# githomin/sketches-py

Hardware: AMD Instinct MI355X
Metric: values ingested/sec (node) @1M streams eps=0.01; % of HBM roofline (higher is better)
Workload: dtype f64; 1 GPU; cfg3: 1000000 streams x 1000 values per GPU, eps=0.01, pareto, ingest + quantiles(.5,.9,.99); split=weak, streams_per_gpu=1000000, parallelism=stream-sharded x1, weak: every rank its own batch (no collective)

## Files before the change

### sketches-py_amd/csrc/gk_kernels.hip

```cpp
#include <hip/hip_runtime.h>
#include <hip/hip_ext.h>
#include <stdint.h>
#include <math.h>

#include <algorithm>
#include <atomic>
#include <limits>
#include <type_traits>

#include "gk_dev.h"
#include "gk_launch.h"
#include "gk_query.h"
#include "gk_state.h"
#include "gk_xor.h"

#define GK_PROF_NSEC 12
#ifndef GK_PROF_FIRST
#define GK_PROF_FIRST 1
#endif
#ifdef GK_PROF
__device__ unsigned long long gk_prof_acc[GK_PROF_NSEC];
__device__ __forceinline__ uint32_t gk_cycles() { return (uint32_t)__builtin_amdgcn_s_memtime(); }
#define GK_MARK(L, sec)                                      \
  do {                                                       \
    if (threadIdx.x == 0) {                                  \
      const uint32_t t_ = gk_cycles();                       \
      (L).prof[sec] += (uint32_t)(t_ - (L).prof_t);         \
      (L).prof_t = t_;                                       \
    }                                                        \
  } while (0)
#else
#define GK_MARK(L, sec) do { } while (0)
#endif
#ifdef GK_PROF
struct GKBigProf {
  unsigned long long acc[GK_PROF_NSEC];
  uint32_t t;
};
__device__ __forceinline__ GKBigProf& gk_big_prof() {
  __shared__ GKBigProf p;
  return p;
}
#define GK_BMARK(sec)                                        \
  do {                                                       \
    if (threadIdx.x == 0) {                                  \
      GKBigProf& p_ = gk_big_prof();                         \
      const uint32_t t_ = gk_cycles();                       \
      p_.acc[sec] += (uint32_t)(t_ - p_.t);                  \
      p_.t = t_;                                             \
    }                                                        \
  } while (0)
#define GK_WP_N 16
#define GK_WP_W 8
__device__ unsigned long long gk_wprof_acc[GK_WP_W][GK_WP_N];
struct GKWaveProf {
  unsigned long long acc[GK_WP_W][GK_WP_N];
  uint32_t t[GK_WP_W];
};
__device__ __forceinline__ GKWaveProf& gk_wave_prof() {
  __shared__ GKWaveProf p;
  return p;
}
#define GK_WMARK(pt)                                                   \
  do {                                                                 \
    if ((threadIdx.x & 63) == 0 && (threadIdx.x >> 6) < GK_WP_W) {     \
      GKWaveProf& p_ = gk_wave_prof();                                 \
      const int w_ = threadIdx.x >> 6;                                 \
      const uint32_t t_ = gk_cycles();                                 \
      p_.acc[w_][pt] += (uint32_t)(t_ - p_.t[w_]);                     \
      p_.t[w_] = t_;                                                   \
    }                                                                  \
  } while (0)
#else
#define GK_BMARK(sec) do { } while (0)
#define GK_WMARK(pt) do { } while (0)
#endif

#define GK_KEEP_BIT 0x40000000

__device__ __forceinline__ int gk_threshold(const GKState& st, int64_t n) {
  double t = floor(st.two_eps * (double)(n - 1));
  if (t > (double)GK_T_CLAMP) t = (double)GK_T_CLAMP;
  if (t < -1.0) t = -1.0;
  return (int)t;
}

__device__ __forceinline__ int clampi(int x, int lo, int hi) { return x < lo ? lo : (x > hi ? hi : x); }

__device__ __forceinline__ int clamp0(int x, int m) {
  int r;
  asm("v_med3_i32 %0, %1, 0, %2" : "=v"(r) : "v"(x), "v"(m));
  return r;
}

#define DPP_WAVE_SHR1 0x138
#define DPP_WAVE_SHL1 0x130

__device__ __forceinline__ int32_t wave_incl_max_i32(int32_t v) {
  v = max(v, __builtin_amdgcn_update_dpp(INT_MIN, v, DPP_ROW_SHR(1), 0xf, 0xf, false));
  v = max(v, __builtin_amdgcn_update_dpp(INT_MIN, v, DPP_ROW_SHR(2), 0xf, 0xf, false));
  v = max(v, __builtin_amdgcn_update_dpp(INT_MIN, v, DPP_ROW_SHR(4), 0xf, 0xf, false));
  v = max(v, __builtin_amdgcn_update_dpp(INT_MIN, v, DPP_ROW_SHR(8), 0xf, 0xf, false));
  v = max(v, __builtin_amdgcn_update_dpp(INT_MIN, v, DPP_ROW_BCAST15, 0xa, 0xf, false));
  v = max(v, __builtin_amdgcn_update_dpp(INT_MIN, v, DPP_ROW_BCAST31, 0xc, 0xf, false));
  return v;
}

__device__ __forceinline__ int wave_shr1(int v, int fill) {
  return __builtin_amdgcn_update_dpp(fill, v, DPP_WAVE_SHR1, 0xf, 0xf, false);
}

__device__ __forceinline__ int64_t wave_shr1_i64(int64_t v, int64_t fill) { return dpp64<DPP_WAVE_SHR1, 0xf>(v, fill); }

template <bool GLOBAL>
__device__ __forceinline__ void wsync() {
  if constexpr (GLOBAL) {
    __syncthreads();
  } else {
    __builtin_amdgcn_fence(__ATOMIC_RELEASE, "wavefront");
    __builtin_amdgcn_wave_barrier();
    __builtin_amdgcn_fence(__ATOMIC_ACQUIRE, "wavefront");
  }
}


template <int VPL>
__device__ __forceinline__ void gk_load_flush_values(double (&xv)[VPL], const double* pb, int p,
                                                     const double* xs, int cnt, int lane) {
  if (cnt <= 0) {
#pragma unroll
    for (int r = 0; r < VPL; ++r) xv[r] = 0.0;
    return;
  }
#pragma unroll
  for (int r = 0; r < VPL; ++r) {
    const int ic = min(lane + 64 * r, cnt - 1);
    const double* a = (ic < p) ? pb + ic : xs + (ic - p);
    xv[r] = *a;
  }
#pragma unroll
  for (int r = 0; r < VPL; ++r) xv[r] = (lane + 64 * r < cnt) ? xv[r] : 0.0;
}

struct GKHdrV {
  int32_t cls, slot, pend, E;
  int64_t n, xo, xe;
  double mn, mx;
};

template <bool MINMAX = true>
__device__ __forceinline__ void gk_hdr_issue(GKHdrV& h, const GKState& st, const int64_t* offs, int64_t s) {
  h.cls = st.cls[s];
  h.slot = st.slot[s];
  h.pend = st.pend[s];
  h.E = st.E[s];
  h.n = st.n[s];
  h.xo = offs[s];
  h.xe = offs[s + 1];
  if constexpr (MINMAX) {
    h.mn = st.mn[s];
    h.mx = st.mx[s];
  } else {
    h.mn = h.mx = 0.0;
  }
}

template <bool MINMAX>
__device__ __forceinline__ uint32_t gk_hdr1_issue(const GKState& st, const int64_t* offs, int64_t s, int lane) {
  constexpr int NW = MINMAX ? 14 : 10;
  const uint32_t* p = (const uint32_t*)(st.cls + s);
  if (lane == 1) p = (const uint32_t*)(st.slot + s);
  if (lane == 2) p = (const uint32_t*)(st.pend + s);
  if (lane == 3) p = (const uint32_t*)(st.E + s);
  if (lane >= 4) p = (const uint32_t*)(st.n + s) + (lane - 4);
  if (lane >= 6) p = (const uint32_t*)(offs + s) + (lane - 6);
  if constexpr (MINMAX) {
    if (lane >= 10) p = (const uint32_t*)(st.mn + s) + (lane - 10);
    if (lane >= 12) p = (const uint32_t*)(st.mx + s) + (lane - 12);
  }
  uint32_t w = 0;
  if (lane < NW) w = *p;
  return w;
}
__device__ __forceinline__ int32_t gk_hdr1_word(uint32_t w, int k) { return __builtin_amdgcn_readlane((int)w, k); }
__device__ __forceinline__ int64_t gk_hdr1_dword(uint32_t w, int k) {
  return (int64_t)(((uint64_t)(uint32_t)__builtin_amdgcn_readlane((int)w, k + 1) << 32) |
                   (uint32_t)__builtin_amdgcn_readlane((int)w, k));
}

__device__ __forceinline__ int64_t rfl64(int64_t v) {
  const int lo = __builtin_amdgcn_readfirstlane((int)(uint32_t)(uint64_t)v);
  const int hi = __builtin_amdgcn_readfirstlane((int)(uint32_t)((uint64_t)v >> 32));
  return (int64_t)(((uint64_t)(uint32_t)hi << 32) | (uint32_t)lo);
}

__device__ __forceinline__ GKRec* gk_table_ptr_cs(const GKState& st, int64_t s, int32_t c, int32_t slot) {
  return c == 0 ? st.tab[0] + s * (int64_t)st.cap[0] : st.tab[c] + (int64_t)slot * st.cap[c];
}

#define GK_SORT_LONG_MAX 4096
#ifndef GK_WG_MAX
#define GK_WG_MAX 64
#endif
#ifndef GK_WG_MIN_FLUSHES
#define GK_WG_MIN_FLUSHES 256
#endif
#define GK_WG_CAP 2048
#define GK_WG_PMAX 1024
#ifndef GK_PRESORT_REL
#define GK_PRESORT_REL 3
#endif
#ifndef GK_PRESORT_REL_WG
#define GK_PRESORT_REL_WG 5
#endif

__global__ __launch_bounds__(1024) void k_long_prep(GKState st, const int64_t* __restrict__ offs,
                                                    int32_t* __restrict__ list, int64_t* __restrict__ list_n,
                                                    const int32_t* __restrict__ count,
                                                    int64_t* __restrict__ list_ws, int64_t* __restrict__ list_b0,
                                                    int64_t ws_cap, int64_t* __restrict__ ws_need,
                                                    int32_t* __restrict__ wg_count, int wg_presort,
                                                    int32_t* __restrict__ go) {
  __shared__ uint64_t key[GK_SORT_LONG_MAX];
  const int cnt = *count;
  const int t = threadIdx.x;
  if (cnt > 1 && cnt <= GK_SORT_LONG_MAX) {
    int N = 2;
    while (N < cnt) N <<= 1;
    constexpr uint64_t LMAX = (1ull << 33) - 1;
    for (int i = t; i < N; i += 1024) {
      uint64_t k = ~0ull;
      if (i < cnt) {
        const int64_t s = list[i];
        uint64_t L = (uint64_t)(offs[s + 1] - offs[s]);
        if (L > LMAX) L = LMAX;
        k = ((LMAX - L) << 31) | (uint64_t)s;
      }
      key[i] = k;
    }
    __syncthreads();
    for (int k = 2; k <= N; k <<= 1) {
      for (int j = k >> 1; j > 0; j >>= 1) {
        for (int pp = t; pp < N / 2; pp += 1024) {
          const int i = ((pp & ~(j - 1)) << 1) | (pp & (j - 1));
          const int l = i + j;
          const uint64_t a = key[i], b = key[l];
          if ((a > b) == ((i & k) == 0)) {
            key[i] = b;
            key[l] = a;
          }
        }
        __syncthreads();
      }
    }
    for (int i = t; i < cnt; i += 1024) list[i] = (int32_t)(key[i] & 0x7fffffffu);
    __syncthreads();
  }
  for (int i = t; i < cnt; i += 1024) list_n[i] = st.n0[list[i]];
  if (!list_ws) return;
  __syncthreads();
  __shared__ int64_t part[1024];
  __shared__ unsigned long long nbmax;
  if (t == 0) nbmax = 0;
  __syncthreads();
  const int per = (cnt + 1023) / 1024;
  const int i0 = t * per, i1 = min(i0 + per, cnt);
  for (int i = i0; i < i1; ++i) {
    const int64_t s = list[i];
    int64_t nb = 0;
    if (st.cls[s] == 0) {
      const int64_t L = offs[s + 1] - offs[s];
      const int64_t need = st.P - (list_n[i] % st.P);
      nb = L >= need ? 1 + (L - need) / st.P : 0;
    }
    list_b0[i] = nb;
    atomicMax(&nbmax, (unsigned long long)nb);
  }
  __syncthreads();
  __shared__ int wk;
  if (wg_count) {
    if (t == 0) {
      int k = 0;
      while (k < cnt && k < GK_WG_MAX && list_b0[k] >= GK_WG_MIN_FLUSHES) ++k;
      if (!(st.cap[0] == GK_WG_CAP && st.P <= GK_WG_PMAX)) k = 0;
      *wg_count = k;
      wk = wg_presort ? k : 0;
    }
    __syncthreads();
  }
  const int64_t nb_min = (int64_t)(nbmax / (wg_count ? GK_PRESORT_REL_WG : GK_PRESORT_REL));
  int64_t mine = 0;
  for (int i = i0; i < i1; ++i) {
    if (list_b0[i] < nb_min || (wg_count && i >= wk)) list_b0[i] = 0;
    mine += list_b0[i];
  }
  part[t] = mine;
  __syncthreads();
  if (t == 0) {
    int64_t acc = 0;
    for (int k = 0; k < 1024; ++k) {
      const int64_t v = part[k];
      part[k] = acc;
      acc += v;
    }
    *ws_need = acc * st.P;
    list_b0[cnt] = acc;
  }
  __syncthreads();
  int64_t b = part[t];
  for (int i = i0; i < i1; ++i) {
    const int64_t nb = list_b0[i];
    list_b0[i] = b;
    list_ws[i] = (nb > 0 && (b + nb) * st.P <= ws_cap) ? b * st.P : -1;
    b += nb;
  }
  if (go) {
    __syncthreads();
    if (t == 0) {
      __threadfence();
      __hip_atomic_store(go, 1, __ATOMIC_RELEASE, __HIP_MEMORY_SCOPE_AGENT);
    }
  }
}

#ifndef GK_SL_BCAST
#define GK_SL_BCAST 1024
#endif

#define SL_BCAST_DEPTH 4
#ifndef SL_DEPTH
#define SL_DEPTH 7
#endif
// ... 1863 lines not shown
                                                   unsigned long long* __restrict__ work, int32_t* __restrict__ ctr) {
  const int lane = threadIdx.x;
  const int P = st.P;
  const BigBuf B = big_buf(ws + (size_t)blockIdx.x * ws_bytes, cap, gk_big_np(P));
  if (count_ptr) count = *count_ptr;
  if ((int64_t)blockIdx.x >= count) return;
  for (;;) {
    unsigned long long wv = 0;
    if (lane == 0) wv = atomicAdd(work, 1ull);
    const int64_t w = rfl64((int64_t)wv);
    if (w >= count) break;
    const int64_t s = list ? (int64_t)list[w] : w;
    if (__builtin_amdgcn_readfirstlane(st.cls[s]) != lcls) continue;
    int p = __builtin_amdgcn_readfirstlane(st.pend[s]);
    int E = __builtin_amdgcn_readfirstlane(st.E[s]);
    int64_t n = rfl64(st.n[s]);
    const int64_t xo = rfl64(offs[s]) + ((lcls > 0 && x) ? n - rfl64(st.n0[s]) : 0);
    const int64_t Lx = rfl64(offs[s + 1]) - xo;
    if (Lx <= 0 && !((force == 1 && p > 0) || (force == 2 && n > 0)) && !qs) continue;
    const bool over = !gk_count_ok(st, n + (Lx > 0 ? Lx : 0));
    const double smn = st.mn[s], smx = st.mx[s];
    GKRec* __restrict__ tab = gk_table_ptr(st, s);
    double* __restrict__ pb = st.pbuf + s * (int64_t)st.pmax;
    bool ok = !over && E <= cap - 1;
    if (ok) {
      for (int j = lane; j < E; j += 64) {
        const GKRec rc = tab[j];
        B.tv[0][j] = rc.v;
        B.tg[0][j] = rc.g;
        B.td[0][j] = rc.d;
      }
    }
    wsync<true>();
    int cur = 0;
    int64_t used = 0;
    int64_t need = P - (n % P);
    while (ok && used + need <= Lx) {
      big_load(B, pb, p, x + xo + used, p + (int)need, lane);
      n += need;
      const int nE = big_flush(B, cap, cur, E, p + (int)need, gk_threshold(st, n), lane);
      if (nE < 0) {
        ok = false;
        break;
      }
      E = nE;
      cur ^= 1;
      used += need;
      p = 0;
      need = P;
    }
    if (ok) {
      const int64_t rem = Lx - used;
      if ((force == 1 && p + rem > 0) || force == 2) {
        big_load(B, pb, p, rem > 0 ? x + xo + used : pb, p + (int)rem, lane);
        n += rem;
        const int nE = big_flush(B, cap, cur, E, p + (int)rem, gk_threshold(st, n), lane);
        if (nE < 0) {
          ok = false;
        } else {
          E = nE;
          cur ^= 1;
          p = 0;
        }
      } else {
        for (int64_t i = lane; i < rem; i += 64) pb[p + i] = x[xo + used + i];
        p += (int)rem;
        n += rem;
      }
    }
    if (!ok) {
      if (lane == 0) {
        if (over) {
          atomicAdd(&ctr[GK_CTR_FATAL], 1);
          atomicMax(&ctr[GK_CTR_FATAL + 1], (int)s);
        } else {
          const int k = atomicAdd(ovf_count, 1);
          ovf_list[k] = (int32_t)s;
        }
      }
      wsync<true>();
      continue;
    }
    const double* fv = cur ? B.tv[1] : B.tv[0];
    const int32_t* fg = cur ? B.tg[1] : B.tg[0];
    const int32_t* fd = cur ? B.td[1] : B.td[0];
    if (qs) wave_quantiles<1, 1>(fv, fg, fd, E, n, smn, smx, st, qs, nq, qmode, qout + s * (int64_t)nq, lane);
    for (int j = lane; j < E; j += 64) {
      GKRec rc;
      rc.v = fv[j];
      rc.g = fg[j];
      rc.d = fd[j];
      tab[j] = rc;
    }
    if (lane == 0) {
      st.n[s] = n;
      st.E[s] = E;
      st.pend[s] = p;
    }
    wsync<true>();
  }
}

#define SMALL_CAP GK_SMALL_CAP
#define GK_SMALL_LX_MAX (((int64_t)1 << 31) - ((int64_t)1 << 15))
#ifndef GK_SMALL_WAVES
#define GK_SMALL_WAVES 7
#endif
#ifndef GK_SMALL_RANK_MAX
#define GK_SMALL_RANK_MAX 16
#endif
__device__ __forceinline__ void gk_lds_order() { __asm__ volatile("" ::: "memory"); }

#ifndef GK_DUP
#define GK_DUP 0
#endif
#define GK_DUPG(g) ((GK_DUP >> (g)) & 1)
template <typename T>
__device__ __forceinline__ void dup_ld(const T* p) {
  const uint32_t a = (uint32_t)(uintptr_t)p;
  if constexpr (sizeof(T) == 16) {
    __attribute__((ext_vector_type(4))) uint32_t w;
    __asm__ volatile("ds_read_b128 %0, %1\n\ts_waitcnt lgkmcnt(0)" : "=v"(w) : "v"(a) : "memory");
  } else if constexpr (sizeof(T) == 8) {
    __attribute__((ext_vector_type(2))) uint32_t w;
    __asm__ volatile("ds_read_b64 %0, %1\n\ts_waitcnt lgkmcnt(0)" : "=v"(w) : "v"(a) : "memory");
  } else {
    uint32_t w;
    __asm__ volatile("ds_read_b32 %0, %1\n\ts_waitcnt lgkmcnt(0)" : "=v"(w) : "v"(a) : "memory");
  }
}
template <typename T>
__device__ __forceinline__ void dup_st(T* p, T v) {
  static_assert(sizeof(T) == 8, "8-byte stores only");
  unsigned long long u;
  __builtin_memcpy(&u, &v, 8);
  *(volatile unsigned long long*)p = u;
}

__device__ __forceinline__ int pidx(int i) { return i + (i >> 5); }
#define SMALL_TVN (SMALL_CAP + (SMALL_CAP >> 5) + 4)


#define GK_SMALL_TRASH (SMALL_CAP + 1)
static_assert(SMALL_CAP == 128, "k_ingest_small is laid out for the 128-entry class (K = 2 entries per lane)");
template <int VPL>
struct SmallLDS {
  alignas(16) double mv[64 * VPL + 64 + 2];
  alignas(16) double tv[SMALL_TVN];
  alignas(16) int2 tgd[SMALL_CAP + 2];
  union {
    alignas(16) int2 gi[SMALL_TVN];
    int32_t mi[64 * VPL + 2];
  };
#ifdef GK_PROF
  unsigned long long prof[GK_PROF_NSEC];
  uint32_t prof_t;
#endif
};

static_assert(SMALL_CAP + (SMALL_CAP >> 5) + 4 == 136, "gi zeroing covers 136 records");
static_assert(sizeof(int32_t) * (64 * 2 + 2) <= sizeof(int2) * 136, "mi fits in the records");
__device__ __forceinline__ void small_zero_counts(int2* gi, int lane) {
  typedef uint32_t gk_v4u __attribute__((ext_vector_type(4)));
  gk_v4u z;
  __asm__ volatile("v_mov_b64 %0, 0" : "=v"(z.xy));
  __asm__ volatile("v_mov_b64 %0, 0" : "=v"(z.zw));
  int l7 = lane & 7;
  __asm__ volatile("" : "+v"(l7));
  ((gk_v4u*)gi)[lane] = z;
  ((uint2*)gi)[128 + l7] = make_uint2(z.x, z.y);
}

__device__ __forceinline__ void small_pad(double* tv, int E, int lane) {
  tv[pidx(min(E + lane, SMALL_CAP - 1))] = __longlong_as_double(0x7ff0000000000000LL);
}

struct CsDiv {
  int cs;
  uint32_t m;
  __device__ __forceinline__ int div(int a) const { return (int)(__umul24((uint32_t)a, m) >> 23); }
  __device__ __forceinline__ int rem(int a, int q) const { return a - (int)__umul24((uint32_t)q, (uint32_t)cs); }
};

struct CsMagicTable {
  uint32_t m[256];
  constexpr CsMagicTable() : m() {
    for (uint32_t c = 1; c < 256; ++c) m[c] = ((1u << 23) + c - 1u) / c;
  }
};
__constant__ CsMagicTable gk_cs_magic = CsMagicTable();

__device__ __forceinline__ CsDiv make_csdiv(int T) {
  CsDiv c;
  c.cs = T > 1 ? T : 1;
  c.m = c.cs < 256 ? gk_cs_magic.m[c.cs] : 1u;
  return c;
}

__device__ __forceinline__ uint32_t gd_pack(int g, int d) { return __builtin_amdgcn_perm((uint32_t)d, (uint32_t)g, 0x05040100u); }
__device__ __forceinline__ int gd_g(uint32_t w) { return (int)(w & 0xffffu); }
__device__ __forceinline__ int gd_d(uint32_t w) { return (int)(w >> 16); }

template <int VPL, int DUPG = -1>
__device__ __forceinline__ void small_put(SmallLDS<VPL>& L, int pos, double v, int g, int d) {
  L.tv[pidx(pos)] = v;
  L.tgd[pos] = make_int2(g, d);
  if constexpr (DUPG >= 0 && GK_DUPG(DUPG)) {
    dup_st(&L.tv[pidx(pos)], v);
    dup_st(&L.tgd[pos], make_int2(g, d));
  }
}

__device__ __forceinline__ int gi_ob(int x) { return x & 0xff; }
__device__ __forceinline__ int gi_mb(int x) { return (x >> 8) & 0xff; }
__device__ __forceinline__ int gi_k(int x) { return (x >> 16) & 0xff; }
__device__ __forceinline__ int gi_m(int x) { return (int)((uint32_t)x >> 24); }

template <int VPL, bool NOTAIL = false>
__device__ __forceinline__ void small_emit(SmallLDS<VPL>& L, bool in_gap, const CsDiv& cd, double x, int2 gi,
                                           int rk, bool valid) {
  const int k = gi_k(gi.x);
  if constexpr (NOTAIL) {
    small_put<VPL, 8>(L, (valid && rk >= k) ? gi_ob(gi.x) + rk - k : GK_SMALL_TRASH, x, 1, gi.y);
    return;
  }
  const int q = cd.div(rk);
  const int rr = cd.rem(rk, q);
  const int pos = gi_ob(gi.x) + (in_gap ? rk - k : q);
  const bool keep = valid && (in_gap ? rk >= k : (rr == cd.cs - 1 || rk == gi_m(gi.x) - 1));
  small_put<VPL, 8>(L, keep ? pos : GK_SMALL_TRASH, x, in_gap ? 1 : rr + 1, in_gap ? gi.y : 0);
}

template <int J>
__device__ __forceinline__ int lane_xor_i32(int v, int lane) {
  return lane_xor_dpp<J>(v, lane);
}

template <int J>
__device__ __forceinline__ double lane_xor_f64(double v, int lane) {
  typedef int gk_v2i __attribute__((ext_vector_type(2)));
  const gk_v2i a = __builtin_bit_cast(gk_v2i, v);
  gk_v2i r;
  r.x = lane_xor_i32<J>(a.x, lane);
  r.y = lane_xor_i32<J>(a.y, lane);
  return __builtin_bit_cast(double, r);
}

template <int X, int LB>
__device__ __forceinline__ void cx_stage2(double (&a)[2], int lane) {
  const bool lower = (lane & LB) == 0;
  if constexpr (X == LB && (X == 16 || X == 32)) {
    typedef int gk_v2i __attribute__((ext_vector_type(2)));
#pragma unroll
    for (int r = 0; r < 2; ++r) {
      const gk_v2i v = __builtin_bit_cast(gk_v2i, a[r]);
      gk_v2i A, B;
      if constexpr (X == 16) {
        const auto lo = __builtin_amdgcn_permlane16_swap(v.x, v.x, false, false);
        const auto hi = __builtin_amdgcn_permlane16_swap(v.y, v.y, false, false);
        A.x = (int)lo[0]; B.x = (int)lo[1]; A.y = (int)hi[0]; B.y = (int)hi[1];
      } else {
        const auto lo = __builtin_amdgcn_permlane32_swap(v.x, v.x, false, false);
        const auto hi = __builtin_amdgcn_permlane32_swap(v.y, v.y, false, false);
        A.x = (int)lo[0]; B.x = (int)lo[1]; A.y = (int)hi[0]; B.y = (int)hi[1];
      }
      const double da = __builtin_bit_cast(double, A), db = __builtin_bit_cast(double, B);
      a[r] = ((db < da) == lower) ? db : da;
    }
    return;
  }
#pragma unroll
  for (int r = 0; r < 2; ++r) {
    const double p = lane_xor_f64<X>(a[r], lane);
    const bool take = (p < a[r]) == lower;
    a[r] = take ? p : a[r];
  }
}

template <int J>
__device__ __forceinline__ void half_cleaners2(double (&a)[2], int lane) {
  cx_stage2<J, J>(a, lane);
  if constexpr (J > 1) half_cleaners2<J / 2>(a, lane);
}

template <int KB>
__device__ __forceinline__ void sort_runs2(double (&a)[2], int lane) {
  if constexpr (KB > 2) sort_runs2<KB / 2>(a, lane);
  cx_stage2<KB - 1, KB / 2>(a, lane);
  if constexpr (KB >= 4) half_cleaners2<KB / 4>(a, lane);
}

__device__ __forceinline__ void sort128_2(double (&a)[2], int lane) {
  sort_runs2<64>(a, lane);
  {
    const double p0 = lane_xor_f64<63>(a[1], lane);
    const double p1 = lane_xor_f64<63>(a[0], lane);
    const bool t0 = p0 < a[0];
    const bool t1 = a[1] < p1;
    a[0] = t0 ? p0 : a[0];
    a[1] = t1 ? p1 : a[1];
  }
  half_cleaners2<32>(a, lane);
}

#define GK_PS_R 16

// ... 586 lines not shown
template <int VPL>
__device__ __attribute__((noinline)) double small_quantiles(SmallLDS<VPL>& L, int E, int64_t n, double mn, double mx,
                                                            double inv_eps, double eps, double qv, int qe, int qmode,
                                                            int lane) {
  const bool valid = (qv >= 0.0 && qv <= 1.0);
  if (n == 0 || E == 0) return gk_nan();
  if ((double)n < inv_eps)
    return valid ? percentile_linear_at(E, qv, [&](int i) { return L.tv[pidx(i)]; }) : gk_nan();
  const double spread_d = floor(eps * (double)(n - 1));
  const int myi = n < ((int64_t)1 << 30) ? small_rank_count<int32_t>(L, E, n, spread_d, qv, qe, lane)
                                         : small_rank_count<int64_t>(L, E, n, spread_d, qv, qe, lane);
  if (!valid) return gk_nan();
  if (myi == 0) return mn;
  if (myi < E) return L.tv[pidx(myi - 1)];
  return (qmode == 0) ? mx : L.tv[pidx(E - 1)];
}

#ifndef GK_FS_DEPTH
#define GK_FS_DEPTH 2
#endif
#define GK_SWORK_IDX 128
#ifndef GK_FS_LAG_DEFAULT
#define GK_FS_LAG_DEFAULT 256
#endif
#ifndef GK_FS_DRAIN
#define GK_FS_DRAIN 1
#endif
#ifndef GK_FS_SPIN_MAX
#define GK_FS_SPIN_MAX (1 << 16)
#endif

template <int DEPTH = GK_FS_DEPTH>
__device__ __forceinline__ void fused_stats_role(const GKState& st, const double* __restrict__ x,
                                                 const int64_t* __restrict__ offs,
                                                 unsigned long long* __restrict__ work, int part, int lgp,
                                                 int64_t count, int pace, int lag, int lane) {
  const int64_t pbeg = (count * part) >> lgp, pend = (count * (part + 1)) >> lgp;
  const int64_t nb = (pend - pbeg + 63) / 64;
  unsigned long long* __restrict__ swork = work + GK_SWORK_IDX + 16 * part;
  unsigned long long* __restrict__ iwork = work + 16 * part;
  const double2* __restrict__ dummy = (const double2*)st.rtab;
  for (;;) {
    unsigned long long v = 0;
    if (lane == 0) v = atomicAdd(swork, 1ull);
    const int64_t b = rfl64((int64_t)v);
    if (b >= nb) break;
    if (pace) {
      const int64_t want = min((b + 1) * 64 + (int64_t)lag, pend - pbeg);
      for (int spin = 0; spin < GK_FS_SPIN_MAX; ++spin) {
        unsigned long long got = 0;
        if (lane == 0) got = __hip_atomic_load(iwork, __ATOMIC_RELAXED, __HIP_MEMORY_SCOPE_AGENT);
        if (rfl64((int64_t)got) >= want) break;
        __builtin_amdgcn_s_sleep(8);
      }
    }
    const int64_t s = (int64_t)((int)(pbeg + b * 64) + lane);
    const bool live = s < pend;
    const int64_t xo = live ? offs[s] : 0;
    int64_t rem = live ? offs[s + 1] - xo : 0;
    if (rem > GK_STATS_LONG) rem = 0;
    const bool act = rem > 0;
    int64_t n = 0;
    double mn = 0, mx = 0, sm = 0, av = 0;
    if (act) {
      n = st.n0[s];
      mn = st.mn[s];
      mx = st.mx[s];
      sm = st.sum[s];
      av = st.avg[s];
    }
    const int64_t peel = (act && (((uintptr_t)(x + xo)) & 8)) ? 1 : 0;
    if (peel) {
      gk_stat_step(x[xo], n, sm, av, mn, mx);
      --rem;
    }
    const double* p = x + xo + peel;
    const int64_t nch = rem / 8;
    int64_t maxch = nch;
#pragma unroll
    for (int o = 32; o > 0; o >>= 1) maxch = max(maxch, (int64_t)__shfl_xor(maxch, o, 64));
    const double2* __restrict__ p2 = (const double2*)p;
    int64_t nlo = act ? n : INT64_MAX, nhi = act ? n : INT64_MIN;
#pragma unroll
    for (int o = 32; o > 0; o >>= 1) {
      nlo = min(nlo, (int64_t)__shfl_xor(nlo, o, 64));
      nhi = max(nhi, (int64_t)__shfl_xor(nhi, o, 64));
    }
    const int64_t nu = rfl64(nlo);
    const bool uni = nu == rfl64(nhi) && nu >= 0 && nu + 8 * maxch + 8 < st.rtab_n;
    double2 ring[DEPTH][4];
#pragma unroll
    for (int d = 0; d < DEPTH; ++d) {
      const double2* src = (d < nch) ? p2 + d * 4 : dummy;
#pragma unroll
      for (int j = 0; j < 4; ++j) ring[d][j] = src[j];
    }
    auto walk = [&](auto tab) {
      constexpr bool TAB = decltype(tab)::value;
      for (int64_t c0 = 0; c0 < maxch; c0 += DEPTH) {
#pragma unroll
        for (int d = 0; d < DEPTH; ++d) {
          const int64_t c = c0 + d;
          if (c < nch) {
            const double* __restrict__ rt = st.rtab + (nu + 8 * c + 1);
#pragma unroll
            for (int k = 0; k < 8; ++k) {
              const double v = (k & 1) ? ring[d][k >> 1].y : ring[d][k >> 1].x;
              const double rc = TAB ? rt[k] : 1.0 / (double)(n + 1 + k);
              sm = sm + v;
              av = av + (v - av) * rc;
              if (v < mn) mn = v;
              if (v > mx) mx = v;
            }
            n += 8;
          }
          const int64_t nx = c + DEPTH;
          const double2* src = (nx < nch) ? p2 + nx * 4 : dummy;
#pragma unroll
          for (int j = 0; j < 4; ++j) ring[d][j] = src[j];
        }
      }
    };
    if (uni) walk(std::true_type{});
    else walk(std::false_type{});
    const int tail = (int)(rem - nch * 8);
    for (int k = 0; k < tail; ++k) gk_stat_step(p[nch * 8 + k], n, sm, av, mn, mx);
    if (act) {
      st.mn[s] = mn;
      st.mx[s] = mx;
      st.sum[s] = sm;
      st.avg[s] = av;
    }
  }
}

#ifdef GK_TIMELINE
#define GK_TL_MAXS (1 << 20)
#define GK_TL_MAXW 16384
__device__ unsigned long long gk_tl_wave[5 * GK_TL_MAXW];
__device__ unsigned long long gk_tl_sbeg[GK_TL_MAXS];
__device__ unsigned long long gk_tl_send[GK_TL_MAXS];
#endif
template <int VPL, bool FS, int W = GK_SMALL_WAVES>
__global__ __launch_bounds__(64, W) void k_ingest_small(GKState st, const double* __restrict__ x,
                                                     const int64_t* __restrict__ offs, int64_t count, int force,
                                                     int32_t* __restrict__ ovf_count, int32_t* __restrict__ ovf_list,
                                                     const double* __restrict__ qs, int nq,
                                                     double* __restrict__ qout, int qmode,
                                                     unsigned long long* __restrict__ work, int nstat,
                                                     int fs_pace, int fs_lag) {
  __shared__ __attribute__((aligned(16))) SmallLDS<VPL> L;
  const int lane = threadIdx.x;
  const int P = st.P;
#ifdef GK_PROF
  if (lane == 0) {
    for (int i = 0; i < GK_PROF_NSEC; ++i) L.prof[i] = 0;
    L.prof_t = gk_cycles();
  }
#endif
  uint32_t hv = 0;
#ifndef GK_WORK_PARTS
#define GK_WORK_PARTS 8
#endif
#ifndef GK_WORK_CHUNK
#define GK_WORK_CHUNK 2
#endif
  static_assert((GK_WORK_PARTS & (GK_WORK_PARTS - 1)) == 0, "a power of two");
  int lgp = 0;
  while ((2 << lgp) <= GK_WORK_PARTS && (2u << lgp) <= gridDim.x) ++lgp;
  const int part = (int)(blockIdx.x & ((1u << lgp) - 1u));
#ifdef GK_TIMELINE
  if (lane == 0 && blockIdx.x < GK_TL_MAXW) {
    gk_tl_wave[5 * blockIdx.x] = __builtin_amdgcn_s_memrealtime();
    gk_tl_wave[5 * blockIdx.x + 3] = __builtin_amdgcn_s_memtime();
  }
#endif
  if (FS && (int)blockIdx.x < nstat) fused_stats_role(st, x, offs, work, part, lgp, count, fs_pace, fs_lag, lane);
#ifdef GK_TIMELINE
  if (lane == 0 && blockIdx.x < GK_TL_MAXW) gk_tl_wave[5 * blockIdx.x + 1] = __builtin_amdgcn_s_memrealtime();
#endif
  const int64_t pbeg = (count * part) >> lgp, pend = (count * (part + 1)) >> lgp;
  const double qpre = (qs && lane < nq) ? qs[lane] : 0.0;
  int64_t cur = 0, cend = 0;
  auto grab = [&]() -> int64_t {
    if (cur >= cend) {
      unsigned long long v = 0;
      if (lane == 0) v = atomicAdd(work + 16 * part, (unsigned long long)GK_WORK_CHUNK);
      cur = pbeg + rfl64((int64_t)v);
      cend = min(cur + GK_WORK_CHUNK, pend);
      if (cur >= pend) return count;
    }
    return cur++;
  };
  int64_t w = grab();
  if (w < count) hv = gk_hdr1_issue<!FS>(st, offs, w, lane);
#ifdef GK_PROF
  bool prof_done_any = false;
#endif
  for (; w < count;) {
    const int64_t s = w;
    const int64_t wn = grab();
    const int32_t scls = gk_hdr1_word(hv, 0);
    const int32_t sslot = gk_hdr1_word(hv, 1);
    int p = gk_hdr1_word(hv, 2);
    int E = gk_hdr1_word(hv, 3);
    int64_t n = gk_hdr1_dword(hv, 4);
    const int64_t xo = gk_hdr1_dword(hv, 6);
    const int64_t xe = gk_hdr1_dword(hv, 8);
    const double smn = __longlong_as_double(FS ? GK_QMARK_MIN : gk_hdr1_dword(hv, 10));
    const double smx = __longlong_as_double(FS ? GK_QMARK_MAX : gk_hdr1_dword(hv, 12));
    if (wn < count) hv = gk_hdr1_issue<!FS>(st, offs, wn, lane);
    w = wn;
    if (scls != 0) continue;
#ifdef GK_TIMELINE
    if (lane == 0 && s < GK_TL_MAXS) gk_tl_sbeg[s] = __builtin_amdgcn_s_memrealtime();
#endif
    const int64_t Lx = xe - xo;
    if (Lx <= 0 && !((force == 1 && p > 0) || (force == 2 && n > 0)) && !qs) continue;
    GKRec* __restrict__ tab = gk_table_ptr_cs(st, s, scls, sslot);
    double* __restrict__ pb = st.pbuf + s * (int64_t)st.pmax;
    bool ok = E <= SMALL_CAP - 1 && gk_count_ok(st, n + (Lx > 0 ? Lx : 0)) && Lx < GK_SMALL_LX_MAX;
    if (ok) {
      const int4* __restrict__ t4 = (const int4*)tab;
      int4 rc[SMALL_CAP / 64];
#pragma unroll
      for (int r = 0; r < SMALL_CAP / 64; ++r)
        rc[r] = (lane + 64 * r < E) ? t4[lane + 64 * r] : make_int4(0, 0, 0, 0);
#pragma unroll
      for (int r = 0; r < SMALL_CAP / 64; ++r) {
        const int j = lane + 64 * r;
        if (j < E) {
          L.tv[pidx(j)] = __hiloint2double(rc[r].y, rc[r].x);
          L.tgd[j] = make_int2(rc[r].z, rc[r].w);
        }
      }
      small_pad(L.tv, E, lane);
      small_zero_counts(L.gi, lane);
    }
    wsync<false>();
    GK_MARK(L, 0);

    bool flushed = false;
    bool final_done = false;
    const int L32 = (int)Lx;
    int used = 0;
    const int need0 = P - (int)(n % P);
    int need = need0;
    const double nm1c = (double)(n - 1);
    int fl = 0;
    int tT = 0;
    uint32_t tM = 0;
    auto plan_t = [&]() {
      const int k = min(need0 + (fl + lane) * P, L32);
      tT = (int)(st.two_eps * (nm1c + (double)k));
      const uint32_t cs = (uint32_t)max(tT, 1);
      tM = cs < 256u ? ((1u << 23) + cs - 1u) / cs : 1u;
    };
    const double* const xs = x ? x + xo : pb;
    double xv[VPL];
#pragma unroll
    for (int r = 0; r < VPL; ++r) xv[r] = 0.0;
    while (ok) {
      const bool autof = need <= L32 - used;
      int nadd;
      if (autof) {
        nadd = need;
      } else {
        nadd = L32 - used;
        if (!((force == 1 && p + nadd > 0) || force == 2)) break;
      }
      const int cnt = p + nadd;
      if (!flushed) gk_load_flush_values<VPL>(xv, pb, p, xs, cnt, lane);
      const int nused = used + nadd;
      const int navail = autof ? min(P, L32 - nused) : 0;
      double xn[VPL];
      auto prefetch = [&]() {
        const __amdgpu_buffer_rsrc_t rs =
            __builtin_amdgcn_make_buffer_rsrc((void*)(xs + nused), 0, navail * (int)sizeof(double), 0x00020000);
#pragma unroll
        for (int r = 0; r < VPL; ++r)
          xn[r] = __builtin_bit_cast(double, __builtin_amdgcn_raw_buffer_load_b64(rs, (lane + 64 * r) * 8, 0, 0));
      };
      if ((fl & 63) == 0) plan_t();
      n += nadd;
      const int T = __builtin_amdgcn_readlane(tT, fl & 63);
      CsDiv cd;
      cd.cs = max(T, 1);
      cd.m = (uint32_t)__builtin_amdgcn_readlane((int)tM, fl & 63);
      ++fl;
      GK_MARK(L, (GK_PROF_FIRST == 2 ? !flushed : (GK_PROF_FIRST && !prof_done_any)) ? 11 : 8);
      int nE;
      if constexpr (SMALL_CAP > 128)
        nE = E <= 127 ? flush_small<VPL, 2>(L, E, xv, cnt, T, cd, lane, prefetch)
                      : flush_small<VPL, 4>(L, E, xv, cnt, T, cd, lane, prefetch);
      else
        nE = flush_small<VPL, 2>(L, E, xv, cnt, T, cd, lane, prefetch);
      if (nE < 0) {
        n -= nadd;
        ok = false;
        break;
      }
      E = nE;
      used = nused;
      p = 0;
      need = P;
      flushed = true;
#pragma unroll
      for (int r = 0; r < VPL; ++r) xv[r] = xn[r];
      GK_MARK(L, 10);
      if (!autof) {
        final_done = true;
        break;
      }
    }
    if (ok && !final_done) {
      const int rem = L32 - used;
      if (flushed) {
#pragma unroll
        for (int r = 0; r < VPL; ++r)
          if (lane + 64 * r < rem) pb[lane + 64 * r] = xv[r];
      } else {
        for (int i = lane; i < rem; i += 64) pb[p + i] = xs[used + i];
      }
      p += rem;
      n += rem;
    }
    auto write_back = [&]() {
      double v[2];
      int2 gd[2];
#pragma unroll
      for (int r = 0; r < 2; ++r) {
        v[r] = L.tv[pidx(lane + 64 * r)];
        gd[r] = L.tgd[lane + 64 * r];
      }
#pragma unroll
      for (int r = 0; r < 2; ++r)
        if (lane + 64 * r < E) ((int4*)tab)[lane + 64 * r] = make_int4(__double2loint(v[r]), __double2hiint(v[r]), gd[r].x, gd[r].y);
      if (lane == 0) {
        st.n[s] = n;
        st.E[s] = E;
        st.pend[s] = p;
      }
    };
    if (!ok) {
      if (flushed) write_back();
      if (lane == 0) {
        const int k = atomicAdd(ovf_count, 1);
        ovf_list[k] = (int32_t)s;
      }
      wsync<false>();
      continue;
    }
    if (qs) {
      for (int q0 = 0; q0 < nq; q0 += 64) {
        int ql = lane;
        __asm__ volatile("" : "+v"(ql));
        const double qv = nq <= 64 ? qpre : ((q0 + ql < nq) ? qs[q0 + ql] : 0.0);
        const double r = small_quantiles<VPL>(L, E, n, smn, smx, st.inv_eps, st.eps, qv, min(nq - q0, 64), qmode, lane);
        if (q0 + ql < nq) qout[s * (int64_t)nq + q0 + ql] = r;
      }
    }
    write_back();
    wsync<false>();
    GK_MARK(L, 9);
#ifdef GK_TIMELINE
    if (lane == 0 && s < GK_TL_MAXS) gk_tl_send[s] = __builtin_amdgcn_s_memrealtime();
#endif
#ifdef GK_PROF
    prof_done_any = true;
#endif
  }
  if (FS && GK_FS_DRAIN) fused_stats_role(st, x, offs, work, part, lgp, count, fs_pace, fs_lag, lane);
#ifdef GK_PROF
  if (lane == 0)
    for (int i = 0; i < GK_PROF_NSEC; ++i) atomicAdd(&gk_prof_acc[i], L.prof[i]);
#endif
#ifdef GK_TIMELINE
  if (lane == 0 && blockIdx.x < GK_TL_MAXW) {
    gk_tl_wave[5 * blockIdx.x + 2] = __builtin_amdgcn_s_memrealtime();
    gk_tl_wave[5 * blockIdx.x + 4] = __builtin_amdgcn_s_memtime();
  }
#endif
}

#define GK_MAX_DEV 64
template <typename Q>
static int per_device(std::atomic<int> (&cache)[GK_MAX_DEV], Q query) {
  int dev = 0;
  (void)hipGetDevice(&dev);
  std::atomic<int>& c = cache[(unsigned)dev % GK_MAX_DEV];
  int v = c.load(std::memory_order_relaxed);
  if (v <= 0) {
    v = query(dev);
    if (v <= 0) v = 1;
    c.store(v, std::memory_order_relaxed);
  }
  return v;
}

static int num_cu() {
  static std::atomic<int> cache[GK_MAX_DEV];
  return per_device(cache, [](int dev) {
    hipDeviceProp_t prop;
    return hipGetDeviceProperties(&prop, dev) == hipSuccess && prop.multiProcessorCount > 0 ? prop.multiProcessorCount
                                                                                           : 256;
  });
}

int gk_num_cu() { return num_cu(); }

int gk_wg_early_ok() { return num_cu() >= 2 * GK_WG_MAX; }

template <int CAP, int VPL>
static hipError_t launch_ingest_t(const GKState& st, const double* x, const int64_t* offs,
                                  const int32_t* list, int64_t count, const int32_t* count_ptr, int lcls,
                                  int force, int cap,
                                  unsigned char* ws, size_t ws_bytes, int64_t ws_blocks,
                                  int32_t* ovf_count, int32_t* ovf_list, const GKQuery& q,
                                  unsigned long long* work, const int32_t* prio, const int32_t* prio_count,
                                  const double* psort, const int64_t* prio_ws, const int32_t* prio_skip, hipStream_t stream,
                                  const GKPoolDev& pool, int pmode) {
  if (count <= 0 && !count_ptr) return hipSuccess;
  if (!work) return hipErrorInvalidValue;
  int64_t grid;
  if (CAP > 0) {
    static std::atomic<int> occ_cache[GK_MAX_DEV];
    const int occ = per_device(occ_cache, [](int) {
      int o = 0;
      (void)hipOccupancyMaxActiveBlocksPerMultiprocessor(&o, k_ingest<CAP, VPL>, 64, 0);
      return o;
    });
    grid = (int64_t)num_cu() * occ;
  } else {
    grid = ws_blocks;
  }
  if (!prio && !count_ptr && grid > count) grid = count;
  if (grid < 1) grid = 1;
  hipLaunchKernelGGL((k_ingest<CAP, VPL>), dim3((unsigned)grid), dim3(64), 0, stream, st, x, offs, list,
                     count, count_ptr, lcls, force, cap, ws, ws_bytes, ovf_count, ovf_list, q.qs, q.nq, q.out,
                     q.mode, work, prio, prio_count, psort, prio_ws, prio_skip, pool, pmode);
  return hipGetLastError();
}

template <int CAP>
static hipError_t launch_ingest_vpl(int vpl, const GKState& st, const double* x, const int64_t* offs,
                                    const int32_t* list, int64_t count, const int32_t* count_ptr, int lcls,
                                    int force, int cap, unsigned char* ws,
                                    size_t ws_bytes, int64_t ws_blocks, int32_t* ovf_count, int32_t* ovf_list,
                                    const GKQuery& q, unsigned long long* work, const int32_t* prio,
                                    const int32_t* prio_count, const double* psort, const int64_t* prio_ws, const int32_t* prio_skip,
                                    hipStream_t stream, const GKPoolDev& pool, int pmode) {
#define GK_L(V) launch_ingest_t<CAP, V>(st, x, offs, list, count, count_ptr, lcls, force, cap, ws, ws_bytes, ws_blocks, \
                                        ovf_count, ovf_list, q, work, prio, prio_count, psort, prio_ws, prio_skip, stream, \
                                        pool, pmode)
  switch (vpl) {
    case 1: return GK_L(1);
    case 2: return GK_L(2);
    case 4: return GK_L(4);
    case 8: return GK_L(8);
    case 16: return GK_L(16);
    default: return hipErrorInvalidValue;
  }
#undef GK_L
}

template <int VPL>
static hipError_t launch_ingest_small(const GKState& st, const double* x, const int64_t* offs, const int32_t* list,
                                      int64_t count, int force, int32_t* ovf_count, int32_t* ovf_list,
                                      const GKQuery& q, unsigned long long* work, int fused_stats,
                                      hipStream_t stream, hipEvent_t ev0, hipEvent_t ev1) {
  if (count <= 0) return hipSuccess;
  if (!work) return hipErrorInvalidValue;
  const bool fs_launch = fused_stats > 0 && x && !list;
  static std::atomic<int> occ_cache[2][2][GK_MAX_DEV];
  auto occ_of = [&](bool fs, bool w6) -> int {
    return per_device(occ_cache[fs][w6], [fs, w6](int) {
      int o = 0;
      if (fs) {
        if (w6) (void)hipOccupancyMaxActiveBlocksPerMultiprocessor(&o, k_ingest_small<VPL, true, 6>, 64, 0);
        else (void)hipOccupancyMaxActiveBlocksPerMultiprocessor(&o, k_ingest_small<VPL, true>, 64, 0);
      } else {
        if (w6) (void)hipOccupancyMaxActiveBlocksPerMultiprocessor(&o, k_ingest_small<VPL, false, 6>, 64, 0);
        else (void)hipOccupancyMaxActiveBlocksPerMultiprocessor(&o, k_ingest_small<VPL, false>, 64, 0);
      }
      return o;
    });
  };
  auto full_grid = [&](bool w6) -> int64_t {
    int64_t g = (int64_t)num_cu() * occ_of(fs_launch, w6);
    return std::max<int64_t>(1, std::min<int64_t>(g, count));
  };
  static const int w_env = getenv("GK_SMALL_W") ? atoi(getenv("GK_SMALL_W")) : 0;
  static const int few_rounds = getenv("GK_FEW_ROUNDS") ? atoi(getenv("GK_FEW_ROUNDS")) : 4;
  int64_t grid = full_grid(false);
  const int64_t rounds7 = (count + grid - 1) / grid;
  const bool w6 = w_env ? w_env == 6 : (GK_SMALL_WAVES != 6 && rounds7 <= few_rounds);
  if (w6) grid = full_grid(true);
  int nstat = 0;
  if (fs_launch) {
    const int64_t want = std::max<int64_t>(1, (int64_t)num_cu() * fused_stats / 8);
    nstat = (int)(grid < want ? grid : want);
  }
  const int pace = nstat > 0 && grid >= 4 * (int64_t)nstat && grid >= 8 * GK_WORK_PARTS ? 1 : 0;
  static const int lag = getenv("GK_FS_LAG") ? atoi(getenv("GK_FS_LAG")) : GK_FS_LAG_DEFAULT;
  if (list) return hipErrorInvalidValue;
#define GK_SMALL_LAUNCH(FS_, W_)                                                                              \
  hipExtLaunchKernelGGL((k_ingest_small<VPL, FS_, W_>), dim3((unsigned)grid), dim3(64), 0, stream, ev0, ev1, 0, st, x, \
                        offs, count, force, ovf_count, ovf_list, q.qs, q.nq, q.out, q.mode, work, nstat, pace, lag)
  if (nstat > 0) {
    if (w6) GK_SMALL_LAUNCH(true, 6);
    else GK_SMALL_LAUNCH(true, GK_SMALL_WAVES);
  } else {
    if (w6) GK_SMALL_LAUNCH(false, 6);
    else GK_SMALL_LAUNCH(false, GK_SMALL_WAVES);
// ... 135 lines not shown
```

Before: 181.9 billion values/s.

## Software-pipeline stream headers, work grabs and first value chunk across iterations

Restructures the small-ingest loop so the next stream's work-counter atomic, header load and first block of input values are issued while the current stream is still being processed, hiding their latency. Header base pointers and quantile probes are staged in LDS, and work indices are narrowed to 32-bit atomics. Skipped streams no longer `continue` early, so the control flow changes. This adds register pressure and more complex state that could cost occupancy, and the 32-bit atomic on a 64-bit counter assumes the stream count fits in an int.

```diff
diff --git a/sketches-py_amd/csrc/gk_kernels.hip b/sketches-py_amd/csrc/gk_kernels.hip
--- a/sketches-py_amd/csrc/gk_kernels.hip
+++ b/sketches-py_amd/csrc/gk_kernels.hip
@@ -166,18 +166,35 @@
 }
 
 template <bool MINMAX>
-__device__ __forceinline__ uint32_t gk_hdr1_issue(const GKState& st, const int64_t* offs, int64_t s, int lane) {
+__device__ __forceinline__ const uint32_t* gk_hdr1_base(const GKState& st, const int64_t* offs, int lane) {
+  const uint32_t* p = (const uint32_t*)st.cls;
+  if (lane == 1) p = (const uint32_t*)st.slot;
+  if (lane == 2) p = (const uint32_t*)st.pend;
+  if (lane == 3) p = (const uint32_t*)st.E;
+  if (lane >= 4) p = (const uint32_t*)st.n + (lane - 4);
+  if (lane >= 6) p = (const uint32_t*)offs + (lane - 6);
+  if constexpr (MINMAX) {
+    if (lane >= 10) p = (const uint32_t*)st.mn + (lane - 10);
+    if (lane >= 12) p = (const uint32_t*)st.mx + (lane - 12);
+  }
+  return p;
+}
+template <bool MINMAX>
+__device__ __forceinline__ uint32_t gk_hdr1_issue_args(const GKState& st, const int64_t* offs, int64_t s, int lane) {
   constexpr int NW = MINMAX ? 14 : 10;
-  const uint32_t* p = (const uint32_t*)(st.cls + s);
-  if (lane == 1) p = (const uint32_t*)(st.slot + s);
-  if (lane == 2) p = (const uint32_t*)(st.pend + s);
-  if (lane == 3) p = (const uint32_t*)(st.E + s);
-  if (lane >= 4) p = (const uint32_t*)(st.n + s) + (lane - 4);
-  if (lane >= 6) p = (const uint32_t*)(offs + s) + (lane - 6);
-  if constexpr (MINMAX) {
-    if (lane >= 10) p = (const uint32_t*)(st.mn + s) + (lane - 10);
-    if (lane >= 12) p = (const uint32_t*)(st.mx + s) + (lane - 12);
-  }
+  const uint32_t* p = gk_hdr1_base<MINMAX>(st, offs, lane) + (lane >= 4 ? 2 * s : s);
+  uint32_t w = 0;
+  if (lane < NW) w = *p;
+  return w;
+}
+#define GK_HDR1_LANES 16
+template <bool MINMAX>
+__device__ __forceinline__ uint32_t gk_hdr1_issue(const unsigned long long* hb, int64_t s, int lane) {
+  constexpr int NW = MINMAX ? 14 : 10;
+  int l = lane & (GK_HDR1_LANES - 1);
+  __asm__ volatile("" : "+v"(l));
+  typedef const uint32_t __attribute__((address_space(1))) * gptr;
+  gptr p = (gptr)(uintptr_t)hb[l] + (l >= 4 ? 2 * s : s);
   uint32_t w = 0;
   if (lane < NW) w = *p;
   return w;
@@ -2347,6 +2364,8 @@
     alignas(16) int2 gi[SMALL_TVN];
     int32_t mi[64 * VPL + 2];
   };
+  unsigned long long hb[GK_HDR1_LANES];
+  double qp[64];
 #ifdef GK_PROF
   unsigned long long prof[GK_PROF_NSEC];
   uint32_t prof_t;
@@ -3239,6 +3258,8 @@
   __shared__ __attribute__((aligned(16))) SmallLDS<VPL> L;
   const int lane = threadIdx.x;
   const int P = st.P;
+  L.qp[lane] = (qs && lane < nq) ? qs[lane] : 0.0;
+  if (lane < GK_HDR1_LANES) L.hb[lane] = (unsigned long long)(uintptr_t)gk_hdr1_base<!FS>(st, offs, lane);
 #ifdef GK_PROF
   if (lane == 0) {
     for (int i = 0; i < GK_PROF_NSEC; ++i) L.prof[i] = 0;
@@ -3266,47 +3287,84 @@
 #ifdef GK_TIMELINE
   if (lane == 0 && blockIdx.x < GK_TL_MAXW) gk_tl_wave[5 * blockIdx.x + 1] = __builtin_amdgcn_s_memrealtime();
 #endif
-  const int64_t pbeg = (count * part) >> lgp, pend = (count * (part + 1)) >> lgp;
-  const double qpre = (qs && lane < nq) ? qs[lane] : 0.0;
-  int64_t cur = 0, cend = 0;
-  auto grab = [&]() -> int64_t {
+  const int pbeg = (int)((count * part) >> lgp), pend = (int)((count * (part + 1)) >> lgp);
+  const int nstr = (int)count;
+  int cur = 0, cend = 0;
+  uint32_t gv = 0;
+  bool gwait = false;
+  auto grab_issue = [&]() {
     if (cur >= cend) {
-      unsigned long long v = 0;
-      if (lane == 0) v = atomicAdd(work + 16 * part, (unsigned long long)GK_WORK_CHUNK);
-      cur = pbeg + rfl64((int64_t)v);
+      typedef uint32_t __attribute__((address_space(1))) * gptr;
+      gptr wp = (gptr)(work + 16 * part);
+      __asm__ volatile("" : "+v"(wp));
+      gv = 0;
+      if (lane == 0) gv = __hip_atomic_fetch_add(wp, (uint32_t)GK_WORK_CHUNK, __ATOMIC_RELAXED, __HIP_MEMORY_SCOPE_AGENT);
+      gwait = true;
+    }
+  };
+  auto grab_take = [&]() -> int {
+    if (gwait) {
+      gwait = false;
+      cur = pbeg + __builtin_amdgcn_readfirstlane((int)gv);
       cend = min(cur + GK_WORK_CHUNK, pend);
-      if (cur >= pend) return count;
+      if (cur >= pend) return nstr;
     }
     return cur++;
   };
-  int64_t w = grab();
-  if (w < count) hv = gk_hdr1_issue<!FS>(st, offs, w, lane);
+  auto hdr_issue = [&](int sn) -> uint32_t {
+    if constexpr (VPL > 1) return gk_hdr1_issue<!FS>(L.hb, sn, lane);
+    else return gk_hdr1_issue_args<!FS>(st, offs, sn, lane);
+  };
+  int32_t h_cls = 0, h_slot = 0, h_p = 0, h_E = 0;
+  int64_t h_n = 0, h_xo = 0, h_xe = 0, h_mn = 0, h_mx = 0;
+  auto hdr_read = [&]() {
+    h_cls = gk_hdr1_word(hv, 0);
+    h_slot = gk_hdr1_word(hv, 1);
+    h_p = gk_hdr1_word(hv, 2);
+    h_E = gk_hdr1_word(hv, 3);
+    h_n = gk_hdr1_dword(hv, 4);
+    h_xo = gk_hdr1_dword(hv, 6);
+    h_xe = gk_hdr1_dword(hv, 8);
+    h_mn = FS ? GK_QMARK_MIN : gk_hdr1_dword(hv, 10);
+    h_mx = FS ? GK_QMARK_MAX : gk_hdr1_dword(hv, 12);
+  };
+  grab_issue();
+  int w = grab_take();
+  if (w < nstr) {
+    hv = hdr_issue(w);
+    hdr_read();
+    grab_issue();
+  }
 #ifdef GK_PROF
   bool prof_done_any = false;
 #endif
-  for (; w < count;) {
+  double xv[VPL];
+  bool pre = false;
+  for (; w < nstr;) {
     const int64_t s = w;
-    const int64_t wn = grab();
-    const int32_t scls = gk_hdr1_word(hv, 0);
-    const int32_t sslot = gk_hdr1_word(hv, 1);
-    int p = gk_hdr1_word(hv, 2);
-    int E = gk_hdr1_word(hv, 3);
-    int64_t n = gk_hdr1_dword(hv, 4);
-    const int64_t xo = gk_hdr1_dword(hv, 6);
-    const int64_t xe = gk_hdr1_dword(hv, 8);
-    const double smn = __longlong_as_double(FS ? GK_QMARK_MIN : gk_hdr1_dword(hv, 10));
-    const double smx = __longlong_as_double(FS ? GK_QMARK_MAX : gk_hdr1_dword(hv, 12));
-    if (wn < count) hv = gk_hdr1_issue<!FS>(st, offs, wn, lane);
-    w = wn;
-    if (scls != 0) continue;
+    auto next_hdr = [&]() {
+      w = grab_take();
+      if (w < nstr) hv = hdr_issue(w);
+    };
+    const bool had = pre;
+    pre = false;
+    const int32_t scls = h_cls;
+    const int32_t sslot = h_slot;
+    int p = h_p;
+    int E = h_E;
+    int64_t n = h_n;
+    const int64_t xo = h_xo;
+    const int64_t xe = h_xe;
+    const double smn = __longlong_as_double(h_mn);
+    const double smx = __longlong_as_double(h_mx);
+    const int64_t Lx = xe - xo;
+    const bool run = scls == 0 && !(Lx <= 0 && !((force == 1 && p > 0) || (force == 2 && n > 0)) && !qs);
 #ifdef GK_TIMELINE
-    if (lane == 0 && s < GK_TL_MAXS) gk_tl_sbeg[s] = __builtin_amdgcn_s_memrealtime();
-#endif
-    const int64_t Lx = xe - xo;
-    if (Lx <= 0 && !((force == 1 && p > 0) || (force == 2 && n > 0)) && !qs) continue;
+    if (run && lane == 0 && s < GK_TL_MAXS) gk_tl_sbeg[s] = __builtin_amdgcn_s_memrealtime();
+#endif
     GKRec* __restrict__ tab = gk_table_ptr_cs(st, s, scls, sslot);
     double* __restrict__ pb = st.pbuf + s * (int64_t)st.pmax;
-    bool ok = E <= SMALL_CAP - 1 && gk_count_ok(st, n + (Lx > 0 ? Lx : 0)) && Lx < GK_SMALL_LX_MAX;
+    bool ok = run && E <= SMALL_CAP - 1 && gk_count_ok(st, n + (Lx > 0 ? Lx : 0)) && Lx < GK_SMALL_LX_MAX;
     if (ok) {
       const int4* __restrict__ t4 = (const int4*)tab;
       int4 rc[SMALL_CAP / 64];
@@ -3325,13 +3383,14 @@
       small_zero_counts(L.gi, lane);
     }
     wsync<false>();
+    next_hdr();
     GK_MARK(L, 0);
 
     bool flushed = false;
     bool final_done = false;
     const int L32 = (int)Lx;
     int used = 0;
-    const int need0 = P - (int)(n % P);
+    const int need0 = ok ? P - (int)(n % P) : P;
     int need = need0;
     const double nm1c = (double)(n - 1);
     int fl = 0;
@@ -3344,9 +3403,10 @@
       tM = cs < 256u ? ((1u << 23) + cs - 1u) / cs : 1u;
     };
     const double* const xs = x ? x + xo : pb;
-    double xv[VPL];
-#pragma unroll
-    for (int r = 0; r < VPL; ++r) xv[r] = 0.0;
+    if (!had) {
+#pragma unroll
+      for (int r = 0; r < VPL; ++r) xv[r] = 0.0;
+    }
     while (ok) {
       const bool autof = need <= L32 - used;
       int nadd;
@@ -3357,7 +3417,14 @@
         if (!((force == 1 && p + nadd > 0) || force == 2)) break;
       }
       const int cnt = p + nadd;
-      if (!flushed) gk_load_flush_values<VPL>(xv, pb, p, xs, cnt, lane);
+      if (!flushed) {
+        if (had) {
+#pragma unroll
+          for (int r = 0; r < VPL; ++r) xv[r] = (lane + 64 * r < cnt) ? xv[r] : 0.0;
+        } else {
+          gk_load_flush_values<VPL>(xv, pb, p, xs, cnt, lane);
+        }
+      }
       const int nused = used + nadd;
       const int navail = autof ? min(P, L32 - nused) : 0;
       double xn[VPL];
@@ -3412,6 +3479,7 @@
       p += rem;
       n += rem;
     }
+    if (w < nstr) hdr_read();
     auto write_back = [&]() {
       double v[2];
       int2 gd[2];
@@ -3429,24 +3497,36 @@
         st.pend[s] = p;
       }
     };
-    if (!ok) {
+    if (run && !ok) {
       if (flushed) write_back();
       if (lane == 0) {
         const int k = atomicAdd(ovf_count, 1);
         ovf_list[k] = (int32_t)s;
       }
       wsync<false>();
-      continue;
-    }
-    if (qs) {
+    }
+    if (ok && qs) {
       for (int q0 = 0; q0 < nq; q0 += 64) {
         int ql = lane;
         __asm__ volatile("" : "+v"(ql));
-        const double qv = nq <= 64 ? qpre : ((q0 + ql < nq) ? qs[q0 + ql] : 0.0);
+        const double qv = nq <= 64 ? L.qp[ql] : ((q0 + ql < nq) ? qs[q0 + ql] : 0.0);
         const double r = small_quantiles<VPL>(L, E, n, smn, smx, st.inv_eps, st.eps, qv, min(nq - q0, 64), qmode, lane);
         if (q0 + ql < nq) qout[s * (int64_t)nq + q0 + ql] = r;
       }
     }
+    if (w < nstr) {
+      grab_issue();
+      const int64_t nLx = h_xe - h_xo;
+      if (x && h_cls == 0 && h_p == 0 && nLx > 0 && nLx < GK_SMALL_LX_MAX) {
+        const __amdgpu_buffer_rsrc_t rs = __builtin_amdgcn_make_buffer_rsrc(
+            (void*)(x + h_xo), 0, (int)min((int64_t)P, nLx) * (int)sizeof(double), 0x00020000);
+#pragma unroll
+        for (int r = 0; r < VPL; ++r)
+          xv[r] = __builtin_bit_cast(double, __builtin_amdgcn_raw_buffer_load_b64(rs, (lane + 64 * r) * 8, 0, 0));
+        pre = true;
+      }
+    }
+    if (!ok) continue;
     write_back();
     wsync<false>();
     GK_MARK(L, 9);
```

Result: slower. 177.4 billion values/s (-2.5%).
